# tencent-ailab/pika

Hardware: NVIDIA H100
Metric: utterances/sec RNN-T train step (T=1000,U=150,V=6k) (higher is better)
Workload: dtype bf16

## Files before the change

### pika_b200/csrc/lstm_seq.cu

```cuda
#include <cooperative_groups.h>

#include "../../include/pika_b200.h"
#include "common.cuh"

namespace pk {
void count_launch();

constexpr int LS_HJ = 8;
constexpr int LS_MB = 32;
constexpr int LS_THREADS = 256;
constexpr int LS_PAD = 8;

PK_DEVICE void mma_bf16_16816(float (&c)[4], uint32_t a0, uint32_t a1, uint32_t a2, uint32_t a3, uint32_t b0, uint32_t b1) {
    asm volatile(
        "mma.sync.aligned.m16n8k16.row.col.f32.bf16.bf16.f32 {%0,%1,%2,%3}, {%4,%5,%6,%7}, {%8,%9}, {%0,%1,%2,%3};"
        : "+f"(c[0]), "+f"(c[1]), "+f"(c[2]), "+f"(c[3])
        : "r"(a0), "r"(a1), "r"(a2), "r"(a3), "r"(b0), "r"(b1));
}
PK_DEVICE uint4 ldcg16(const void* p) {
    uint4 r;
    asm volatile("ld.global.cg.v4.u32 {%0,%1,%2,%3}, [%4];" : "=r"(r.x), "=r"(r.y), "=r"(r.z), "=r"(r.w) : "l"(p));
    return r;
}
PK_DEVICE void bulk_g2s(void* smem_dst, const void* gsrc, uint32_t bytes, uint64_t* bar) {
    asm volatile("cp.async.bulk.shared::cluster.global.mbarrier::complete_tx::bytes [%0], [%1], %2, [%3];" ::"r"(smem_u32(smem_dst)),
                 "l"(gsrc), "r"(bytes), "r"(smem_u32(bar))
                 : "memory");
}
PK_DEVICE void bulk_g2s_mc(void* smem_dst, const void* gsrc, uint32_t bytes, uint64_t* bar, uint16_t mask) {
    asm volatile("cp.async.bulk.shared::cluster.global.mbarrier::complete_tx::bytes.multicast::cluster [%0], [%1], %2, [%3], %4;" ::"r"(
                     smem_u32(smem_dst)),
                 "l"(gsrc), "r"(bytes), "r"(smem_u32(bar)), "h"(mask)
                 : "memory");
}
PK_DEVICE void fence_proxy_async_all() { asm volatile("fence.proxy.async;" ::: "memory"); }

PK_DEVICE void grid_barrier(unsigned int* counter, unsigned int step_index, unsigned int nct) {
    const unsigned int target = nct * step_index;
    __syncthreads();
    if (threadIdx.x == 0) {
        asm volatile("red.release.gpu.global.add.u32 [%0], 1;" ::"l"(counter) : "memory");
        unsigned int seen;
        do {
            asm volatile("ld.acquire.gpu.global.u32 %0, [%1];" : "=r"(seen) : "l"(counter) : "memory");
        } while (seen < target);
    }
    __syncthreads();
}
PK_DEVICE float sigm(float x) { return 1.f / (1.f + __expf(-x)); }

PK_DEVICE void load_lens(const int* lens, int B, int U, int* len_s, int* steps_s) {
    if (threadIdx.x < 32) {
        int L = 0;
        if ((int)threadIdx.x < B) L = lens ? min(max(lens[threadIdx.x], 0), U) : U;
        len_s[threadIdx.x] = L;
        int m = L;
#pragma unroll
        for (int o = 16; o > 0; o >>= 1) m = max(m, __shfl_xor_sync(0xffffffffu, m, o));
        if (threadIdx.x == 0) *steps_s = m;
    }
}

struct LsDir {
    int d;
    bool rev;
    int j0;
    unsigned nct;
};
PK_DEVICE LsDir ls_dir(int H, int reverse) {
    LsDir r;
    r.nct = (unsigned)(H / LS_HJ);
    r.d = (int)(blockIdx.x / r.nct);
    r.rev = gridDim.x > r.nct ? r.d == 1 : reverse != 0;
    r.j0 = (int)(blockIdx.x - r.d * r.nct) * LS_HJ;
    return r;
}

template <typename T>
__global__ void __launch_bounds__(LS_THREADS, 1) lstm_seq_fwd_kernel(const float* __restrict__ gx, const __nv_bfloat16* __restrict__ w_hh,
                                                                     T* __restrict__ out, int ldo, __nv_bfloat16* hx, float* __restrict__ gates_save,
                                                                     float* __restrict__ cs, const int* __restrict__ lens, int B, int Bt, int U,
                                                                     int H, int reverse, unsigned int* counter) {
    extern __shared__ __align__(16) uint8_t sm_raw[];
    const int P = H + LS_PAD;
    __nv_bfloat16* w_s = reinterpret_cast<__nv_bfloat16*>(sm_raw);
    __nv_bfloat16* h_s = w_s + 32 * P;
    float* g_s = reinterpret_cast<float*>(h_s + 32 * P);
    const int tid = threadIdx.x, warp = tid >> 5, lane = tid & 31;
    const LsDir dir = ls_dir(H, reverse);
    const int j0 = dir.j0;
    gx += (long long)dir.d * Bt * U * 4 * H;
    w_hh += (long long)dir.d * 4 * H * H;
    out += dir.d * H;
    hx += (long long)dir.d * 2 * LS_MB * H;
    gates_save += (long long)dir.d * U * Bt * 4 * H;
    cs += (long long)dir.d * U * Bt * H;
    counter += dir.d * 32;
    __shared__ int len_s[LS_MB], steps_s;
    load_lens(lens, B, U, len_s, &steps_s);
    const int vec_per_row = H / 8;
    for (int i = tid; i < 32 * vec_per_row; i += LS_THREADS) {
        const int r = i / vec_per_row, v = i - r * vec_per_row;
        const int grow = (r >> 3) * H + j0 + (r & 7);
        *reinterpret_cast<uint4*>(w_s + r * P + v * 8) = *reinterpret_cast<const uint4*>(w_hh + (long long)grow * H + v * 8);
    }
    const int cb = tid >> 3, cj = tid & 7;
    float c_state = 0.f;
    const int mt = warp & 1, nt = warp >> 1;
    const int g = lane >> 2, tq = lane & 3;
    __shared__ __align__(8) uint64_t h_bar;
    if (tid == 0) { mbar_init(&h_bar, 1); mbar_fence_init(); }
    uint32_t h_phase = 0;
    const uint32_t cn = cluster_nctarank(), cr = cluster_ctarank();
    const uint16_t cmask = (uint16_t)((1u << cn) - 1u);
    __syncthreads();
    if (cn > 1) cluster_sync_all();
    const int S = steps_s, L = len_s[cb];
    for (int s = 0; s < S; ++s) {
        const bool active = s < L;
        const int t = dir.rev ? L - 1 - s : s;
        float acc[4] = {0.f, 0.f, 0.f, 0.f};
        float gx_i = 0.f, gx_f = 0.f, gx_g = 0.f, gx_o = 0.f;
        if (active) {
            const float* gxr = gx + ((long long)cb * U + t) * 4 * H + j0 + cj;
            gx_i = __ldg(gxr); gx_f = __ldg(gxr + H); gx_g = __ldg(gxr + 2 * H); gx_o = __ldg(gxr + 3 * H);
        }
        if (s > 0) {
            const __nv_bfloat16* src = hx + (long long)((s - 1) & 1) * LS_MB * H;
            if (warp == 0) {
                fence_proxy_async_all();
                if (lane == 0) mbar_arrive_expect_tx(&h_bar, 32u * (uint32_t)H * 2u);
                __syncwarp();
                if (cn == 1) bulk_g2s(h_s + lane * P, src + (long long)lane * H, (uint32_t)H * 2u, &h_bar);
                else if ((lane % cn) == cr) bulk_g2s_mc(h_s + lane * P, src + (long long)lane * H, (uint32_t)H * 2u, &h_bar, cmask);
            }
            mbar_wait(&h_bar, h_phase);
            h_phase ^= 1;
            const __nv_bfloat16* ar0 = h_s + (mt * 16 + g) * P + 2 * tq;
            const __nv_bfloat16* ar1 = ar0 + 8 * P;
            const __nv_bfloat16* br = w_s + (nt * 8 + g) * P + 2 * tq;
            float acc1[4] = {0.f, 0.f, 0.f, 0.f}, acc2[4] = {0.f, 0.f, 0.f, 0.f}, acc3[4] = {0.f, 0.f, 0.f, 0.f};
            auto mma_at = [&](float (&c)[4], int k0) {
                const uint32_t a0 = *reinterpret_cast<const uint32_t*>(ar0 + k0), a1 = *reinterpret_cast<const uint32_t*>(ar1 + k0);
                const uint32_t a2 = *reinterpret_cast<const uint32_t*>(ar0 + k0 + 8), a3 = *reinterpret_cast<const uint32_t*>(ar1 + k0 + 8);
                const uint32_t b0 = *reinterpret_cast<const uint32_t*>(br + k0), b1 = *reinterpret_cast<const uint32_t*>(br + k0 + 8);
                mma_bf16_16816(c, a0, a1, a2, a3, b0, b1);
            };
#pragma unroll 4
            for (int k0 = 0; k0 < H; k0 += 64) {
                mma_at(acc, k0);
                mma_at(acc1, k0 + 16);
                mma_at(acc2, k0 + 32);
                mma_at(acc3, k0 + 48);
            }
#pragma unroll
            for (int e = 0; e < 4; ++e) acc[e] = (acc[e] + acc1[e]) + (acc2[e] + acc3[e]);
        }
        g_s[(mt * 16 + g) * 33 + nt * 8 + 2 * tq] = acc[0];
        g_s[(mt * 16 + g) * 33 + nt * 8 + 2 * tq + 1] = acc[1];
        g_s[(mt * 16 + g + 8) * 33 + nt * 8 + 2 * tq] = acc[2];
        g_s[(mt * 16 + g + 8) * 33 + nt * 8 + 2 * tq + 1] = acc[3];
        __syncthreads();
        if (active) {
            const float gi = sigm(g_s[cb * 33 + cj] + gx_i);
            const float gf = sigm(g_s[cb * 33 + 8 + cj] + gx_f);
            const float gg = tanhf(g_s[cb * 33 + 16 + cj] + gx_g);
            const float go = sigm(g_s[cb * 33 + 24 + cj] + gx_o);
            c_state = gf * c_state + gi * gg;
            const float hv = go * tanhf(c_state);
            out[((long long)cb * U + t) * ldo + j0 + cj] = from_f32<T>(hv);
            hx[(long long)(s & 1) * LS_MB * H + (long long)cb * H + j0 + cj] = __float2bfloat16_rn(hv);
            float* gs = gates_save + ((long long)t * Bt + cb) * 4 * H + j0 + cj;
            gs[0] = gi; gs[H] = gf; gs[2 * H] = gg; gs[3 * H] = go;
            cs[((long long)t * Bt + cb) * H + j0 + cj] = c_state;
        } else {
            hx[(long long)(s & 1) * LS_MB * H + (long long)cb * H + j0 + cj] = __float2bfloat16_rn(0.f);
            if (cb < B) out[((long long)cb * U + s) * ldo + j0 + cj] = from_f32<T>(0.f);
        }
        if (s + 1 < S) grid_barrier(counter, (unsigned int)(s + 1), dir.nct);
    }
    if (cb < B)
        for (int t = S; t < U; ++t) out[((long long)cb * U + t) * ldo + j0 + cj] = from_f32<T>(0.f);
}

template <typename T>
__global__ void __launch_bounds__(LS_THREADS, 1) lstm_seq_bwd_kernel(const T* __restrict__ dout, int ldo, const float* __restrict__ gates_save,
                                                                     const float* __restrict__ cs, const __nv_bfloat16* __restrict__ w_hh,
                                                                     __nv_bfloat16* dG, const __nv_bfloat16* zrow, const int* __restrict__ lens,
                                                                     int B, int Bt, int U, int H, int reverse, unsigned int* counter) {
    extern __shared__ __align__(16) uint8_t sm_raw[];
    const int G4 = 4 * H;
    const int PW = G4 + LS_PAD;
    const int KQ = G4 / 4;
    const int PD = KQ + LS_PAD;
    __nv_bfloat16* wt_s = reinterpret_cast<__nv_bfloat16*>(sm_raw);
    __nv_bfloat16* d_s = wt_s + LS_HJ * PW;
    float* r_s = reinterpret_cast<float*>(d_s + 2 * 32 * PD);
    __shared__ __align__(8) uint64_t q_bar[2];
    const int tid = threadIdx.x, warp = tid >> 5, lane = tid & 31;
    const LsDir dir = ls_dir(H, reverse);
    const int j0 = dir.j0;
    dout += dir.d * H;
    gates_save += (long long)dir.d * U * Bt * G4;
    cs += (long long)dir.d * U * Bt * H;
    w_hh += (long long)dir.d * G4 * H;
    dG += (long long)dir.d * U * Bt * G4;
    counter += dir.d * 32;
    __shared__ int len_s[LS_MB], steps_s;
    load_lens(lens, B, U, len_s, &steps_s);
    for (int i = tid; i < G4 * LS_HJ; i += LS_THREADS) {
        const int r = i / LS_HJ, jj = i - r * LS_HJ;
        wt_s[jj * PW + r] = w_hh[(long long)r * H + j0 + jj];
    }
    for (int i = tid; i < 2 * 32 * PD / 8; i += LS_THREADS) reinterpret_cast<uint4*>(d_s)[i] = make_uint4(0, 0, 0, 0);
    for (int i = tid; i < 4 * 32 * 9; i += LS_THREADS) r_s[i] = 0.f;
    if (tid == 0) { mbar_init(&q_bar[0], 1); mbar_init(&q_bar[1], 1); mbar_fence_init(); }
    const int cb = tid >> 3, cj = tid & 7;
    float dc_state = 0.f;
    const int mt = warp & 1, kg = warp >> 1;
    const int g = lane >> 2, tq = lane & 3;
    uint32_t q_phase[2] = {0, 0};
    const uint32_t cn = cluster_nctarank(), cr = cluster_ctarank();
    const uint16_t cmask = (uint16_t)((1u << cn) - 1u);
    __syncthreads();
    if (cn > 1) cluster_sync_all();
    const int S = steps_s, L = len_s[cb];
    if (cb < B)
        for (int t = S; t < U; ++t) {
            __nv_bfloat16* d = dG + ((long long)t * Bt + cb) * G4 + j0 + cj;
            d[0] = d[H] = d[2 * H] = d[3 * H] = __float2bfloat16_rn(0.f);
        }
    const int Lr = len_s[lane];
    for (int s = S - 1; s >= 0; --s) {
        const bool active = s < L;
        const int t = dir.rev ? L - 1 - s : s;
        float pgi = 0.f, pgf = 0.f, pgg = 0.f, pgo = 0.f, pc = 0.f, pcp = 0.f, pdo = 0.f;
        if (active) {
            const int j = j0 + cj;
            const int tp = dir.rev ? t + 1 : t - 1;
            const float* gs = gates_save + ((long long)t * Bt + cb) * G4 + j;
            pgi = __ldg(gs); pgf = __ldg(gs + H); pgg = __ldg(gs + 2 * H); pgo = __ldg(gs + 3 * H);
            pc = __ldg(cs + ((long long)t * Bt + cb) * H + j);
            pcp = s > 0 ? __ldg(cs + ((long long)tp * Bt + cb) * H + j) : 0.f;
            pdo = to_f32<T>(dout[((long long)cb * U + t) * ldo + j]);
        }
        if (s < S - 1) {
            const int tn = dir.rev ? Lr - 2 - s : s + 1;
            const __nv_bfloat16* src = s + 1 < Lr ? dG + ((long long)tn * Bt + lane) * G4 : zrow;
            auto issue = [&](int qtr) {
                if (warp == 0) {
                    fence_proxy_async_all();
                    if (lane == 0) mbar_arrive_expect_tx(&q_bar[qtr & 1], (uint32_t)B * (uint32_t)KQ * 2u);
                    __syncwarp();
                    __nv_bfloat16* dst = d_s + ((qtr & 1) * 32 + lane) * PD;
                    const __nv_bfloat16* from = src + qtr * KQ;
                    if (lane < B) {
                        if (cn == 1) bulk_g2s(dst, from, (uint32_t)KQ * 2u, &q_bar[qtr & 1]);
                        else if ((lane % cn) == cr) bulk_g2s_mc(dst, from, (uint32_t)KQ * 2u, &q_bar[qtr & 1], cmask);
                    }
                }
            };
            issue(0);
            issue(1);
            float acc[4] = {0.f, 0.f, 0.f, 0.f}, accb[4] = {0.f, 0.f, 0.f, 0.f}, accc[4] = {0.f, 0.f, 0.f, 0.f}, accd[4] = {0.f, 0.f, 0.f, 0.f};
            const int kspan = KQ / 4;
            for (int qtr = 0; qtr < 4; ++qtr) {
                mbar_wait(&q_bar[qtr & 1], q_phase[qtr & 1]);
                q_phase[qtr & 1] ^= 1;
                const __nv_bfloat16* ar0 = d_s + ((qtr & 1) * 32 + mt * 16 + g) * PD + kg * kspan + 2 * tq;
                const __nv_bfloat16* ar1 = ar0 + 8 * PD;
                const __nv_bfloat16* br = wt_s + g * PW + qtr * KQ + kg * kspan + 2 * tq;
                auto mma_at = [&](float (&c)[4], int k0) {
                    const uint32_t a0 = *reinterpret_cast<const uint32_t*>(ar0 + k0), a1 = *reinterpret_cast<const uint32_t*>(ar1 + k0);
                    const uint32_t a2 = *reinterpret_cast<const uint32_t*>(ar0 + k0 + 8), a3 = *reinterpret_cast<const uint32_t*>(ar1 + k0 + 8);
                    const uint32_t b0 = *reinterpret_cast<const uint32_t*>(br + k0), b1 = *reinterpret_cast<const uint32_t*>(br + k0 + 8);
                    mma_bf16_16816(c, a0, a1, a2, a3, b0, b1);
                };
                int k0 = 0;
#pragma unroll 4
                for (; k0 + 64 <= kspan; k0 += 64) {
                    mma_at(acc, k0);
                    mma_at(accb, k0 + 16);
                    mma_at(accc, k0 + 32);
                    mma_at(accd, k0 + 48);
                }
                for (; k0 < kspan; k0 += 16) mma_at(acc, k0);
                if (qtr + 2 < 4) {
                    if (cn == 1) __syncthreads();
                    else cluster_sync_all();
                    issue(qtr + 2);
                }
            }
#pragma unroll
            for (int e = 0; e < 4; ++e) acc[e] = (acc[e] + accb[e]) + (accc[e] + accd[e]);
            float* r_k = r_s + kg * 32 * 9;
            r_k[(mt * 16 + g) * 9 + 2 * tq] = acc[0];
            r_k[(mt * 16 + g) * 9 + 2 * tq + 1] = acc[1];
            r_k[(mt * 16 + g + 8) * 9 + 2 * tq] = acc[2];
            r_k[(mt * 16 + g + 8) * 9 + 2 * tq + 1] = acc[3];
        }
        __syncthreads();
        if (active) {
            const int j = j0 + cj;
            const float gi = pgi, gf = pgf, gg = pgg, go = pgo, c = pc, cp = pcp;
            const float* r_c = r_s + cb * 9 + cj;
            const float dh = pdo + (((r_c[0] + r_c[32 * 9]) + r_c[2 * 32 * 9]) + r_c[3 * 32 * 9]);
            const float tc = tanhf(c);
            const float dc = dh * go * (1.f - tc * tc) + dc_state;
            __nv_bfloat16* d = dG + ((long long)t * Bt + cb) * G4 + j;
            d[0] = __float2bfloat16_rn(dc * gg * gi * (1.f - gi));
            d[H] = __float2bfloat16_rn(dc * cp * gf * (1.f - gf));
            d[2 * H] = __float2bfloat16_rn(dc * gi * (1.f - gg * gg));
            d[3 * H] = __float2bfloat16_rn(dh * tc * go * (1.f - go));
            dc_state = dc * gf;
        } else if (cb < B) {
            __nv_bfloat16* d = dG + ((long long)s * Bt + cb) * G4 + j0 + cj;
            d[0] = d[H] = d[2 * H] = d[3 * H] = __float2bfloat16_rn(0.f);
        }
        if (s > 0) grid_barrier(counter, (unsigned int)(S - s), dir.nct);
    }
}
}

using namespace pk;

static int lstm_launch(const void* fn, int grid, int smem, void** args, cudaStream_t st, int* cluster_cache) {
    cudaLaunchConfig_t cfg = {};
    cfg.gridDim = dim3(grid); cfg.blockDim = dim3(LS_THREADS); cfg.dynamicSmemBytes = smem; cfg.stream = st;
    cudaLaunchAttribute attr[2];
    attr[0].id = cudaLaunchAttributeCooperative; attr[0].val.cooperative = 1;
    if (*cluster_cache == 0) {
        int pick = 1;
        for (int cs = 8; cs >= 2; cs >>= 1) {
            if (grid % cs) continue;
            attr[1].id = cudaLaunchAttributeClusterDimension; attr[1].val.clusterDim.x = cs; attr[1].val.clusterDim.y = 1; attr[1].val.clusterDim.z = 1;
            cfg.attrs = attr; cfg.numAttrs = 2;
            int ncl = 0;
            if (cudaOccupancyMaxActiveClusters(&ncl, fn, &cfg) == cudaSuccess && ncl * cs >= grid) { pick = cs; break; }
            (void)cudaGetLastError();
        }
        *cluster_cache = pick;
    }
    attr[1].id = cudaLaunchAttributeClusterDimension; attr[1].val.clusterDim.x = *cluster_cache; attr[1].val.clusterDim.y = 1; attr[1].val.clusterDim.z = 1;
    cfg.attrs = attr; cfg.numAttrs = 2;
    PK_CHECK_CUDA(cudaLaunchKernelExC(&cfg, fn, args));
    return 0;
}
static inline bool aligned16(const void* p) { return (reinterpret_cast<uintptr_t>(p) & 15) == 0; }
static int lstm_seq_check(int B, int U, int H, int n_dir, int ldo) {
    PK_CHECK_ARG(B >= 1, "empty batch");
    PK_CHECK_ARG(U >= 1, "U must be >= 1");
    PK_CHECK_ARG(n_dir == 1 || n_dir == 2, "n_dir must be 1 or 2");
    PK_CHECK_ARG(H >= 64 && H % 64 == 0 && n_dir * H / LS_HJ <= num_sms(), "H must be a multiple of 64 with n_dir * H/8 <= #SMs");
    PK_CHECK_ARG(ldo >= n_dir * H, "ldo must be >= n_dir * H");
    return 0;
}
static int* lstm_cluster_slot(int (*cache)[2][64], int fl, int n_dir, int H) { return &cache[fl][n_dir - 1][(H / 64) & 63]; }

extern "C" long long pk_lstm_seq_workspace_bytes(int H) { return 2ll * LS_MB * H * 2 + 256 + 4ll * H * 2; }

extern "C" int pk_lstm_seq_fwd_ex(const float* gx, const void* w_hh_bf16, void* out, int out_dtype, int ldo, float* gates_save, float* cs,
                                  const int* lens, int B, int U, int H, int n_dir, int reverse, void* ws, void* stream) {
    int rc = lstm_seq_check(B, U, H, n_dir, ldo);
    if (rc) return rc;
    PK_CHECK_ARG(aligned16(w_hh_bf16) && aligned16(ws), "pk_lstm_seq_fwd_ex: w_hh, ws must be 16-byte aligned");
    cudaStream_t st = reinterpret_cast<cudaStream_t>(stream);
    unsigned int* counter = reinterpret_cast<unsigned int*>(ws);
    __nv_bfloat16* hx = reinterpret_cast<__nv_bfloat16*>(reinterpret_cast<unsigned char*>(ws) + 256);
    const int smem = 2 * 32 * (H + LS_PAD) * 2 + 32 * 33 * 4;
    const __nv_bfloat16* w = reinterpret_cast<const __nv_bfloat16*>(w_hh_bf16);
    const void* fn = out_dtype == PK_BF16 ? (const void*)lstm_seq_fwd_kernel<__nv_bfloat16> : (const void*)lstm_seq_fwd_kernel<float>;
    PK_CHECK_CUDA(cudaFuncSetAttribute(fn, cudaFuncAttributeMaxDynamicSharedMemorySize, smem));
    const size_t es = out_dtype == PK_BF16 ? 2 : 4;
    const int grid = n_dir * H / LS_HJ;
    static int cluster_f[2][2][64] = {};
    for (int b0 = 0; b0 < B; b0 += LS_MB) {
        int nb = B - b0 < LS_MB ? B - b0 : LS_MB, Bt = B;
        const float* gx_c = gx + (long long)b0 * U * 4 * H;
        void* out_c = reinterpret_cast<unsigned char*>(out) + (size_t)b0 * U * ldo * es;
        float* gs_c = gates_save + (long long)b0 * 4 * H;
        float* cs_c = cs + (long long)b0 * H;
        const int* lens_c = lens ? lens + b0 : nullptr;
        PK_CHECK_CUDA(cudaMemsetAsync(counter, 0, 256, st));
        void* args[] = {(void*)&gx_c, (void*)&w, (void*)&out_c, (void*)&ldo, (void*)&hx, (void*)&gs_c, (void*)&cs_c, (void*)&lens_c, (void*)&nb,
                        (void*)&Bt, (void*)&U, (void*)&H, (void*)&reverse, (void*)&counter};
        rc = lstm_launch(fn, grid, smem, args, st, lstm_cluster_slot(cluster_f, out_dtype == PK_BF16 ? 0 : 1, n_dir, H));
        if (rc) return rc;
        count_launch();
    }
    return 0;
}
extern "C" int pk_lstm_seq_bwd_ex(const void* dout, int dtype, int ldo, const float* gates_save, const float* cs, const void* w_hh_bf16,
                                  void* dG_bf16, const int* lens, int B, int U, int H, int n_dir, int reverse, void* ws, void* stream) {
    int rc = lstm_seq_check(B, U, H, n_dir, ldo);
    if (rc) return rc;
    PK_CHECK_ARG(aligned16(dG_bf16) && aligned16(ws), "pk_lstm_seq_bwd_ex: dG, ws must be 16-byte aligned");
    cudaStream_t st = reinterpret_cast<cudaStream_t>(stream);
    unsigned int* counter = reinterpret_cast<unsigned int*>(ws);
    const __nv_bfloat16* zrow = reinterpret_cast<const __nv_bfloat16*>(reinterpret_cast<unsigned char*>(ws) + 256 + 2ll * LS_MB * n_dir * H * 2);
    const int G4 = 4 * H;
    const int smem = LS_HJ * (G4 + LS_PAD) * 2 + 2 * 32 * (G4 / 4 + LS_PAD) * 2 + 4 * 32 * 9 * 4;
    const __nv_bfloat16* w = reinterpret_cast<const __nv_bfloat16*>(w_hh_bf16);
    const void* fn = dtype == PK_BF16 ? (const void*)lstm_seq_bwd_kernel<__nv_bfloat16> : (const void*)lstm_seq_bwd_kernel<float>;
    PK_CHECK_CUDA(cudaFuncSetAttribute(fn, cudaFuncAttributeMaxDynamicSharedMemorySize, smem));
    const size_t es = dtype == PK_BF16 ? 2 : 4;
    const int grid = n_dir * H / LS_HJ;
    static int cluster_b[2][2][64] = {};
    for (int b0 = 0; b0 < B; b0 += LS_MB) {
        int nb = B - b0 < LS_MB ? B - b0 : LS_MB, Bt = B;
        const void* dout_c = reinterpret_cast<const unsigned char*>(dout) + (size_t)b0 * U * ldo * es;
        const float* gs_c = gates_save + (long long)b0 * G4;
        const float* cs_c = cs + (long long)b0 * H;
        __nv_bfloat16* dg = reinterpret_cast<__nv_bfloat16*>(dG_bf16) + (long long)b0 * G4;
        const int* lens_c = lens ? lens + b0 : nullptr;
        PK_CHECK_CUDA(cudaMemsetAsync(counter, 0, 256, st));
        void* args[] = {(void*)&dout_c, (void*)&ldo, (void*)&gs_c, (void*)&cs_c, (void*)&w, (void*)&dg, (void*)&zrow, (void*)&lens_c, (void*)&nb,
                        (void*)&Bt, (void*)&U, (void*)&H, (void*)&reverse, (void*)&counter};
        rc = lstm_launch(fn, grid, smem, args, st, lstm_cluster_slot(cluster_b, dtype == PK_BF16 ? 0 : 1, n_dir, H));
        if (rc) return rc;
        count_launch();
    }
    return 0;
}
```

Baseline: 284.2.

## Hold W_hh slice in registers and split K across all warps in LSTM backward

The backward recurrent LSTM kernel now keeps each warp's share of the W_hh column slice in registers as pre-packed MMA B fragments instead of a shared-memory copy. The K dimension is split across all 8 warps, each covering both M tiles, and the eight partial sums are reduced through shared memory. The dG staging buffer grows from two to three slots so three quarters are prefetched up front, leaving only one mid-step sync. The aim is fewer shared-memory loads and less serialisation per timestep, at the cost of many registers (64 per thread for weights), a new H<=1024 limit, and a wider reduction.

```diff
diff --git a/pika_b200/csrc/lstm_seq.cu b/pika_b200/csrc/lstm_seq.cu
--- a/pika_b200/csrc/lstm_seq.cu
+++ b/pika_b200/csrc/lstm_seq.cu
@@ -183,6 +183,11 @@
         for (int t = S; t < U; ++t) out[((long long)cb * U + t) * ldo + j0 + cj] = from_f32<T>(0.f);
 }
 
+constexpr int LS_BW_KS = 8;
+constexpr int LS_BW_SLOTS = 3;
+PK_DEVICE uint32_t bf16_pair(__nv_bfloat16 lo, __nv_bfloat16 hi) {
+    return (uint32_t)__bfloat16_as_ushort(lo) | ((uint32_t)__bfloat16_as_ushort(hi) << 16);
+}
 template <typename T>
 __global__ void __launch_bounds__(LS_THREADS, 1) lstm_seq_bwd_kernel(const T* __restrict__ dout, int ldo, const float* __restrict__ gates_save,
                                                                      const float* __restrict__ cs, const __nv_bfloat16* __restrict__ w_hh,
@@ -190,13 +195,12 @@
                                                                      int B, int Bt, int U, int H, int reverse, unsigned int* counter) {
     extern __shared__ __align__(16) uint8_t sm_raw[];
     const int G4 = 4 * H;
-    const int PW = G4 + LS_PAD;
     const int KQ = G4 / 4;
     const int PD = KQ + LS_PAD;
-    __nv_bfloat16* wt_s = reinterpret_cast<__nv_bfloat16*>(sm_raw);
-    __nv_bfloat16* d_s = wt_s + LS_HJ * PW;
-    float* r_s = reinterpret_cast<float*>(d_s + 2 * 32 * PD);
-    __shared__ __align__(8) uint64_t q_bar[2];
+    const int nks = KQ / 16;
+    __nv_bfloat16* d_s = reinterpret_cast<__nv_bfloat16*>(sm_raw);
+    float* r_s = reinterpret_cast<float*>(d_s + LS_BW_SLOTS * 32 * PD);
+    __shared__ __align__(8) uint64_t q_bar[LS_BW_SLOTS];
     const int tid = threadIdx.x, warp = tid >> 5, lane = tid & 31;
     const LsDir dir = ls_dir(H, reverse);
     const int j0 = dir.j0;
@@ -208,18 +212,30 @@
     counter += dir.d * 32;
     __shared__ int len_s[LS_MB], steps_s;
     load_lens(lens, B, U, len_s, &steps_s);
-    for (int i = tid; i < G4 * LS_HJ; i += LS_THREADS) {
-        const int r = i / LS_HJ, jj = i - r * LS_HJ;
-        wt_s[jj * PW + r] = w_hh[(long long)r * H + j0 + jj];
-    }
-    for (int i = tid; i < 2 * 32 * PD / 8; i += LS_THREADS) reinterpret_cast<uint4*>(d_s)[i] = make_uint4(0, 0, 0, 0);
-    for (int i = tid; i < 4 * 32 * 9; i += LS_THREADS) r_s[i] = 0.f;
-    if (tid == 0) { mbar_init(&q_bar[0], 1); mbar_init(&q_bar[1], 1); mbar_fence_init(); }
+    const int g = lane >> 2, tq = lane & 3;
+    uint32_t wb[4][LS_BW_KS][2];
+#pragma unroll
+    for (int q = 0; q < 4; ++q)
+#pragma unroll
+        for (int i = 0; i < LS_BW_KS; ++i) {
+            const int ks = warp + 8 * i;
+            uint32_t b0 = 0u, b1 = 0u;
+            if (ks < nks) {
+                const __nv_bfloat16* col = w_hh + (long long)(q * KQ + ks * 16 + 2 * tq) * H + j0 + g;
+                b0 = bf16_pair(col[0], col[H]);
+                b1 = bf16_pair(col[8ll * H], col[9ll * H]);
+            }
+            wb[q][i][0] = b0; wb[q][i][1] = b1;
+        }
+    for (int i = tid; i < LS_BW_SLOTS * 32 * PD / 8; i += LS_THREADS) reinterpret_cast<uint4*>(d_s)[i] = make_uint4(0, 0, 0, 0);
+    for (int i = tid; i < 8 * 32 * 9; i += LS_THREADS) r_s[i] = 0.f;
+    if (tid == 0) {
+        for (int k = 0; k < LS_BW_SLOTS; ++k) mbar_init(&q_bar[k], 1);
+        mbar_fence_init();
+    }
     const int cb = tid >> 3, cj = tid & 7;
     float dc_state = 0.f;
-    const int mt = warp & 1, kg = warp >> 1;
-    const int g = lane >> 2, tq = lane & 3;
-    uint32_t q_phase[2] = {0, 0};
+    uint32_t q_phase[LS_BW_SLOTS] = {0, 0, 0};
     const uint32_t cn = cluster_nctarank(), cr = cluster_ctarank();
     const uint16_t cmask = (uint16_t)((1u << cn) - 1u);
     __syncthreads();
@@ -247,64 +263,67 @@
         if (s < S - 1) {
             const int tn = dir.rev ? Lr - 2 - s : s + 1;
             const __nv_bfloat16* src = s + 1 < Lr ? dG + ((long long)tn * Bt + lane) * G4 : zrow;
-            auto issue = [&](int qtr) {
+            auto issue = [&](int qtr, int slot) {
                 if (warp == 0) {
                     fence_proxy_async_all();
-                    if (lane == 0) mbar_arrive_expect_tx(&q_bar[qtr & 1], (uint32_t)B * (uint32_t)KQ * 2u);
+                    if (lane == 0) mbar_arrive_expect_tx(&q_bar[slot], (uint32_t)B * (uint32_t)KQ * 2u);
                     __syncwarp();
-                    __nv_bfloat16* dst = d_s + ((qtr & 1) * 32 + lane) * PD;
+                    __nv_bfloat16* dst = d_s + (slot * 32 + lane) * PD;
                     const __nv_bfloat16* from = src + qtr * KQ;
                     if (lane < B) {
-                        if (cn == 1) bulk_g2s(dst, from, (uint32_t)KQ * 2u, &q_bar[qtr & 1]);
-                        else if ((lane % cn) == cr) bulk_g2s_mc(dst, from, (uint32_t)KQ * 2u, &q_bar[qtr & 1], cmask);
+                        if (cn == 1) bulk_g2s(dst, from, (uint32_t)KQ * 2u, &q_bar[slot]);
+                        else if ((lane % cn) == cr) bulk_g2s_mc(dst, from, (uint32_t)KQ * 2u, &q_bar[slot], cmask);
                     }
                 }
             };
-            issue(0);
-            issue(1);
-            float acc[4] = {0.f, 0.f, 0.f, 0.f}, accb[4] = {0.f, 0.f, 0.f, 0.f}, accc[4] = {0.f, 0.f, 0.f, 0.f}, accd[4] = {0.f, 0.f, 0.f, 0.f};
-            const int kspan = KQ / 4;
+            issue(0, 0);
+            issue(1, 1);
+            issue(2, 2);
+            float acc[2][2][4] = {};
+#pragma unroll
             for (int qtr = 0; qtr < 4; ++qtr) {
-                mbar_wait(&q_bar[qtr & 1], q_phase[qtr & 1]);
-                q_phase[qtr & 1] ^= 1;
-                const __nv_bfloat16* ar0 = d_s + ((qtr & 1) * 32 + mt * 16 + g) * PD + kg * kspan + 2 * tq;
-                const __nv_bfloat16* ar1 = ar0 + 8 * PD;
-                const __nv_bfloat16* br = wt_s + g * PW + qtr * KQ + kg * kspan + 2 * tq;
-                auto mma_at = [&](float (&c)[4], int k0) {
-                    const uint32_t a0 = *reinterpret_cast<const uint32_t*>(ar0 + k0), a1 = *reinterpret_cast<const uint32_t*>(ar1 + k0);
-                    const uint32_t a2 = *reinterpret_cast<const uint32_t*>(ar0 + k0 + 8), a3 = *reinterpret_cast<const uint32_t*>(ar1 + k0 + 8);
-                    const uint32_t b0 = *reinterpret_cast<const uint32_t*>(br + k0), b1 = *reinterpret_cast<const uint32_t*>(br + k0 + 8);
-                    mma_bf16_16816(c, a0, a1, a2, a3, b0, b1);
-                };
-                int k0 = 0;
-#pragma unroll 4
-                for (; k0 + 64 <= kspan; k0 += 64) {
-                    mma_at(acc, k0);
-                    mma_at(accb, k0 + 16);
-                    mma_at(accc, k0 + 32);
-                    mma_at(accd, k0 + 48);
+                const int slot = qtr % LS_BW_SLOTS;
+                mbar_wait(&q_bar[slot], q_phase[slot]);
+                q_phase[slot] ^= 1;
+                const __nv_bfloat16* ab = d_s + (slot * 32 + g) * PD + 2 * tq;
+#pragma unroll
+                for (int i = 0; i < LS_BW_KS; ++i) {
+                    const int ks = warp + 8 * i;
+                    if (ks < nks) {
+#pragma unroll
+                        for (int mt = 0; mt < 2; ++mt) {
+                            const __nv_bfloat16* ar0 = ab + mt * 16 * PD + ks * 16;
+                            const __nv_bfloat16* ar1 = ar0 + 8 * PD;
+                            const uint32_t a0 = *reinterpret_cast<const uint32_t*>(ar0), a1 = *reinterpret_cast<const uint32_t*>(ar1);
+                            const uint32_t a2 = *reinterpret_cast<const uint32_t*>(ar0 + 8), a3 = *reinterpret_cast<const uint32_t*>(ar1 + 8);
+                            mma_bf16_16816(acc[mt][i & 1], a0, a1, a2, a3, wb[qtr][i][0], wb[qtr][i][1]);
+                        }
+                    }
                 }
-                for (; k0 < kspan; k0 += 16) mma_at(acc, k0);
-                if (qtr + 2 < 4) {
+                if (qtr == 0) {
                     if (cn == 1) __syncthreads();
                     else cluster_sync_all();
-                    issue(qtr + 2);
+                    issue(3, 0);
                 }
             }
-#pragma unroll
-            for (int e = 0; e < 4; ++e) acc[e] = (acc[e] + accb[e]) + (accc[e] + accd[e]);
-            float* r_k = r_s + kg * 32 * 9;
-            r_k[(mt * 16 + g) * 9 + 2 * tq] = acc[0];
-            r_k[(mt * 16 + g) * 9 + 2 * tq + 1] = acc[1];
-            r_k[(mt * 16 + g + 8) * 9 + 2 * tq] = acc[2];
-            r_k[(mt * 16 + g + 8) * 9 + 2 * tq + 1] = acc[3];
+            float* r_k = r_s + warp * 32 * 9;
+#pragma unroll
+            for (int mt = 0; mt < 2; ++mt) {
+                r_k[(mt * 16 + g) * 9 + 2 * tq] = acc[mt][0][0] + acc[mt][1][0];
+                r_k[(mt * 16 + g) * 9 + 2 * tq + 1] = acc[mt][0][1] + acc[mt][1][1];
+                r_k[(mt * 16 + g + 8) * 9 + 2 * tq] = acc[mt][0][2] + acc[mt][1][2];
+                r_k[(mt * 16 + g + 8) * 9 + 2 * tq + 1] = acc[mt][0][3] + acc[mt][1][3];
+            }
         }
         __syncthreads();
         if (active) {
             const int j = j0 + cj;
             const float gi = pgi, gf = pgf, gg = pgg, go = pgo, c = pc, cp = pcp;
             const float* r_c = r_s + cb * 9 + cj;
-            const float dh = pdo + (((r_c[0] + r_c[32 * 9]) + r_c[2 * 32 * 9]) + r_c[3 * 32 * 9]);
+            float rec = r_c[0];
+#pragma unroll
+            for (int w = 1; w < 8; ++w) rec += r_c[w * 32 * 9];
+            const float dh = pdo + rec;
             const float tc = tanhf(c);
             const float dc = dh * go * (1.f - tc * tc) + dc_state;
             __nv_bfloat16* d = dG + ((long long)t * Bt + cb) * G4 + j;
@@ -395,11 +414,12 @@
     int rc = lstm_seq_check(B, U, H, n_dir, ldo);
     if (rc) return rc;
     PK_CHECK_ARG(aligned16(dG_bf16) && aligned16(ws), "pk_lstm_seq_bwd_ex: dG, ws must be 16-byte aligned");
+    PK_CHECK_ARG(H <= 8 * LS_BW_KS * 16, "pk_lstm_seq_bwd_ex: H must be <= 1024 (the W_hh slice is held in registers)");
     cudaStream_t st = reinterpret_cast<cudaStream_t>(stream);
     unsigned int* counter = reinterpret_cast<unsigned int*>(ws);
     const __nv_bfloat16* zrow = reinterpret_cast<const __nv_bfloat16*>(reinterpret_cast<unsigned char*>(ws) + 256 + 2ll * LS_MB * n_dir * H * 2);
+    const int smem = LS_BW_SLOTS * 32 * (H + LS_PAD) * 2 + 8 * 32 * 9 * 4;
     const int G4 = 4 * H;
-    const int smem = LS_HJ * (G4 + LS_PAD) * 2 + 2 * 32 * (G4 / 4 + LS_PAD) * 2 + 4 * 32 * 9 * 4;
     const __nv_bfloat16* w = reinterpret_cast<const __nv_bfloat16*>(w_hh_bf16);
     const void* fn = dtype == PK_BF16 ? (const void*)lstm_seq_bwd_kernel<__nv_bfloat16> : (const void*)lstm_seq_bwd_kernel<float>;
     PK_CHECK_CUDA(cudaFuncSetAttribute(fn, cudaFuncAttributeMaxDynamicSharedMemorySize, smem));
```

New measurement: 284.9 (median of 6 runs). Within noise of the previous version (+0.3%).
